# UMich-CURLY/SE3ET

Measured on AMD Instinct MI355X. Metric: point-cloud pairs/sec (fwd), SE3ET-E 5k-pt pairs, higher is better.
Workload: dtype f32

## Files before the change

### include/se3et_hip.h

```cpp
#ifndef SE3ET_HIP_H_
#define SE3ET_HIP_H_

#include <stddef.h>
#include <stdint.h>

#ifdef __cplusplus
extern "C" {
#endif

#define SE3_OK 0
#define SE3_ERR_INVALID_ARG 1
#define SE3_ERR_UNSUPPORTED 2
#define SE3_ERR_LAUNCH 3
#define SE3_ERR_WORKSPACE 4

#define SE3_MAX_BATCH 32
#define SE3_MAX_NEIGHBOR_LIMIT 64

const char* se3_version(void);
const char* se3_last_error(void);
void se3_debug_set_sinkhorn_variant(int variant);
unsigned long long se3_debug_dense_saturated_rows(int reset);
unsigned long long se3_debug_attention_saturated(int reset);
void se3_debug_kernel_timing(int enable);
// ... 34 lines not shown
                                    const int64_t* s_lengths, int batch, const void* tree_host, float radius, int limit,
                                    const int32_t* tie_rows, int64_t num_tie_rows, int max_hits, int64_t* neighbors, int* overflowed);
int64_t se3_debug_std_sort_host(const unsigned long long* keys, int64_t n, int mode);

size_t se3_grid_subsample_workspace_bytes(int64_t n, int batch);
int se3_grid_subsample(const float* points, const float* normals, int64_t n, const int64_t* lengths_host, int batch,
                       float voxel_size, float* s_points, float* s_normals, int64_t* s_lengths, void* workspace,
                       size_t workspace_bytes, void* stream);
int se3_grid_subsample_dev(const float* points, const float* normals, int64_t n_rows, const int64_t* lengths_dev, int batch,
                           float voxel_size, float* s_points, float* s_normals, int64_t* s_lengths, void* workspace,
                           size_t workspace_bytes, void* stream);

int se3_log_sinkhorn_fwd(const float* scores, const uint8_t* row_masks, const uint8_t* col_masks, const float* alpha,
                         int batch, int rows, int cols, int iterations, float inf, float* out, void* stream);
int se3_log_sinkhorn_bwd(const float* scores, const uint8_t* row_masks, const uint8_t* col_masks, const float* alpha,
                         const float* grad_out, int batch, int rows, int cols, int iterations, float inf, float* grad_scores,
                         float* grad_alpha_partial, void* stream);

size_t se3_group_norm_workspace_bytes(int64_t rows, int channels, int groups);
int se3_group_norm_fwd(const float* x, const float* x_bias, const float* residual, const float* weight, const float* bias,
                       int64_t rows, int channels, int groups, float eps, int apply_leaky_relu, float slope, float* out,
                       void* workspace, size_t workspace_bytes, void* stream);

int se3_group_norm_segments_fwd(const float* x, const float* x_bias, const float* residual, const float* weight,
                                const float* bias, int64_t rows, int channels, int groups,
                                const int64_t* segment_row_offsets_host, int num_segments, float eps, int apply_leaky_relu,
                                float slope, float* out, void* workspace, size_t workspace_bytes, void* stream);
size_t se3_group_norm_bwd_workspace_bytes(int channels);
int se3_group_norm_segments_bwd(const float* x, const float* x_bias, const float* residual, const float* weight, const float* bias,
                                const float* grad_out, int64_t rows, int channels, int groups, const int64_t* segment_row_offsets_host,
                                int num_segments, float eps, int apply_leaky_relu, float slope, float* grad_x, float* grad_residual,
                                float* grad_params, void* workspace, size_t workspace_bytes, void* stream);

size_t se3_group_norm_stats_workspace_bytes(int channels);
int se3_group_norm_stats(const float* x, const float* in_affine, float in_slope, const float* x_bias, const float* weight, const float* bias,
                         int64_t rows, int channels, int groups, const int64_t* segment_row_offsets_host, int num_segments, float eps,
                         float* affine_out, void* workspace, size_t workspace_bytes, void* stream);
int se3_group_norm_apply(const float* x, const float* affine_a, float slope_a, const float* affine_b, float slope_b, const float* residual,
                         const float* residual_affine, float final_slope, int64_t rows, int channels,
                         const int64_t* segment_row_offsets_host, int num_segments, int blocked_layout, float* out, void* stream);
int se3_group_norm_apply_amax(const float* x, const float* affine_a, float slope_a, const float* affine_b, float slope_b, const float* residual,
                              const float* residual_affine, float final_slope, int64_t rows, int channels,
                              const int64_t* segment_row_offsets_host, int num_segments, int blocked_layout, float* out, float* amax_out,
                              void* stream);
size_t se3_dense_norm_workspace_bytes(int groups);
int se3_dense_norm_fwd(const float* x, int64_t rows, int in_features, const float* in_affine_a, float in_slope_a, const float* in_affine_b,
                       float in_slope_b, const void* weight_pieces, int out_features, const float* linear_bias, const float* norm_weight,
                       const float* norm_bias, int groups, float eps, const int64_t* segment_row_offsets_host, int num_segments, float* out,
                       float* affine_out, void* workspace, size_t workspace_bytes, void* stream);
int se3_dense_residual_fwd(const float* x, int64_t rows, int in_features, const float* in_affine_a, float in_slope_a, const float* in_affine_b,
                           float in_slope_b, const void* weight_pieces, const float* affine, const float* x2, int in_features2,
                           const void* weight_pieces2, const float* affine2, const float* residual, int out_features, float final_slope,
                           const int64_t* segment_row_offsets_host, int num_segments, float* out, void* stream);
int se3_linear_stream(const float* x, int64_t rows, int in_features, int64_t x_row_stride, const void* weight_pieces, const float* bias,
                      int out_features, int apply_relu, float* out, int64_t out_row_stride, void* stream);
int se3_linear_stream_transposed(const float* x, int64_t rows, int in_features, int64_t x_row_stride, const void* weight_pieces,
                                 const float* bias, int out_features, int block_rows, float* out_t, int64_t ld, void* stream);

int se3_add_layer_norm_fwd(const float* hidden, const float* hidden_bias, const float* residual, const float* weight,
                           const float* bias, int64_t rows, int64_t residual_rows, int channels, float eps, float* out,
                           void* stream);
int se3_add_layer_norm_bwd(const float* hidden, const float* hidden_bias, const float* residual, const float* weight,
                           const float* grad_out, int64_t rows, int64_t residual_rows, int channels, float eps, float* grad_hidden,
                           float* grad_params, void* stream);

size_t se3_linear_weight_pieces_bytes(int out_features, int in_features);
int se3_linear_split_weights_f16(const float* weight, int out_features, int in_features, void* pieces, void* stream);
int se3_linear_f16(const float* x, int64_t rows, int in_features, int64_t x_row_stride, const void* weight_pieces, const float* bias,
                   int out_features, int apply_relu, float* out, int64_t out_row_stride, void* stream);

int se3_gather_rows_padded(const float* x, const int64_t* idx, int64_t n, int64_t m, int64_t width, float* out,
                           void* stream);
int se3_neighbor_max_pool(const float* x, const int64_t* idx, int64_t n, int64_t m, int nn, int64_t width, float* out,
                          void* stream);
int se3_neighbor_max_pool_bwd(const float* x, const int64_t* idx, const float* dout, int64_t n, int64_t m, int nn, int64_t width,
                              float* dx, void* stream);
int se3_anchor_max(const float* x, int num_anchors, int64_t rows, int channels, int64_t anchor_stride, int64_t row_stride,
                   float* out, void* stream);

int se3_kpconv_so3_gather(const float* q_pts, const float* s_pts, const int64_t* idx, const float* x,
                          const float* kernel_points_host, const int64_t* kidx_host, const int64_t* ridx_host, float sigma,
                          int64_t num_queries, int64_t num_support, int num_neighbors, int in_channels, float* G,
                          void* stream);
int se3_kpconv_so3_gather_bwd(const float* q_pts, const float* s_pts, const int64_t* idx, const float* dG,
                              const float* kernel_points_host, const int64_t* kidx_host, const int64_t* ridx_host, float sigma,
                              int64_t num_queries, int64_t num_support, int num_neighbors, int in_channels, float* dx, void* stream);
int se3_kpconv_so3_gather_bwd_fixed(const float* q_pts, const float* s_pts, const int64_t* idx, const float* dG,
                                    const float* kernel_points_host, const int64_t* kidx_host, const int64_t* ridx_host, float sigma,
                                    int64_t num_queries, int64_t num_support, int num_neighbors, int in_channels, const float* max_abs_dG,
                                    long long* dx_fixed, void* stream);
int se3_kpconv_fixed_to_float(const long long* dx_fixed, int64_t count, const float* max_abs_dG, int64_t num_queries, float* dx, void* stream);
int se3_fixed_to_float(const long long* fixed, int64_t count, const float* bound, int64_t terms, int growth, float* out, void* stream);
int se3_neighbor_max_pool_bwd_fixed(const float* x, const int64_t* idx, const float* dout, int64_t n, int64_t m, int nn, int64_t width,
                                    const float* max_abs_dout, long long* dx_fixed, void* stream);
int se3_scatter_add_rows_fixed(const float* g, const int64_t* idx, int64_t n, int64_t m, int64_t width, const float* max_abs_g,
                               long long* dx_fixed, void* stream);
int64_t se3_add_layer_norm_bwd_blocks(int64_t rows);
int se3_add_layer_norm_bwd_partials(const float* hidden, const float* hidden_bias, const float* residual, const float* weight,
                                    const float* grad_out, int64_t rows, int64_t residual_rows, int channels, float eps, float* grad_hidden,
                                    float* grad_params_partials, void* stream);

size_t se3_kpconv_neighbor_table_bytes(int64_t num_queries, int num_neighbors);
int se3_kpconv_neighbor_table(const float* q_pts, const float* s_pts, const int64_t* idx, const float* kernel_points_dev, float sigma,
                              int64_t num_queries, int64_t num_support, int num_neighbors, void* table, size_t table_bytes, void* stream);
size_t se3_kpconv_weight_pieces_bytes(int in_channels, int out_channels);
int se3_kpconv_split_weights_f16(const float* weights, int in_channels, int out_channels, void* pieces, void* stream);
// ... 334 lines not shown
```

### se3et_amd/csrc/dense_norm.hip

```cpp
#include "common.h"
#include "group_norm.h"

namespace {

using f16x8 = __attribute__((ext_vector_type(8))) _Float16;
using f16x4 = __attribute__((ext_vector_type(4))) _Float16;
using f32x16 = __attribute__((ext_vector_type(16))) float;
using f32x4 = __attribute__((ext_vector_type(4))) float;
using u32x4 = __attribute__((ext_vector_type(4))) unsigned;
using i32x4 = __attribute__((ext_vector_type(4))) int;

__device__ unsigned long long g_dense_saturated_rows = 0;

template <int CTRL>
__device__ __forceinline__ float dpp_f32(float v) {
  return __builtin_bit_cast(float, __builtin_amdgcn_update_dpp(0, __builtin_bit_cast(int, v), CTRL, 0xf, 0xf, true));
}

constexpr int kHeaderB = 256;
constexpr int kRowB = 80;

struct DenseArgs {
  const float* x;
  const float* in_affine[2];
// ... 768 lines not shown
    default: plain_launch<4, 1, 1, 1>(a, transposed, grid, st); break;
  }
  SE3_CHECK_LAUNCH("linear_stream");
  return SE3_OK;
}

int linear_stream(const float* x, int64_t rows, int K, int64_t x_rs, const void* weight_pieces, const float* bias, int N, int relu, float* out,
                  int64_t out_rs, int t_rows, int64_t t_ld, void* stream, int seg_channels = 0, int64_t seg_stride = 0) {
  const int64_t lim = (1ll << 29) - 1;
  const bool transposed = t_rows > 0;
  const bool fits = rows >= 0 && x_rs > 0 && rows * x_rs <= lim &&
                    (transposed ? (rows / t_rows) * (int64_t)N * t_ld <= lim : rows * (out_rs > N ? out_rs : (int64_t)N) <= lim);
  if (fits || seg_channels > 0 || !x || !out || N <= 0) return linear_stream_one(x, rows, K, x_rs, weight_pieces, bias, N, relu, out, out_rs, t_rows, t_ld, stream, seg_channels, seg_stride);
  int64_t step;
  if (transposed) {
    SE3_REQUIRE(rows % t_rows == 0 && t_ld >= t_rows, SE3_ERR_INVALID_ARG, "linear_stream: transposed output blocks of %d rows", t_rows);
    const int64_t per_block = std::max((int64_t)t_rows * x_rs, (int64_t)N * t_ld);
    SE3_REQUIRE(per_block <= lim, SE3_ERR_UNSUPPORTED, "linear_stream: one transposed block of %d rows exceeds 2 GB", t_rows);
    step = lim / per_block * t_rows;
  } else {
    SE3_REQUIRE(out_rs >= N, SE3_ERR_INVALID_ARG, "linear_stream: out row stride %lld", (long long)out_rs);
    step = lim / std::max(x_rs, out_rs) / 256 * 256;
    SE3_REQUIRE(step > 0, SE3_ERR_UNSUPPORTED, "linear_stream: row strides %lld / %lld too large", (long long)x_rs, (long long)out_rs);
  }
  for (int64_t r0 = 0; r0 < rows; r0 += step) {
    const int64_t n = std::min(step, rows - r0);
    float* o = transposed ? out + (r0 / t_rows) * (int64_t)N * t_ld : out + r0 * out_rs;
    const int rc = linear_stream_one(x + r0 * x_rs, n, K, x_rs, weight_pieces, bias, N, relu, o, out_rs, t_rows, t_ld, stream);
    if (rc != SE3_OK) return rc;
  }
  return SE3_OK;
}
}

extern "C" int se3_linear_stream(const float* x, int64_t rows, int in_features, int64_t x_row_stride, const void* weight_pieces, const float* bias,
                                 int out_features, int apply_relu, float* out, int64_t out_row_stride, void* stream) {
  return linear_stream(x, rows, in_features, x_row_stride, weight_pieces, bias, out_features, apply_relu, out, out_row_stride, 0, 0, stream);
}

extern "C" int se3_linear_stream_transposed(const float* x, int64_t rows, int in_features, int64_t x_row_stride, const void* weight_pieces,
                                            const float* bias, int out_features, int block_rows, float* out_t, int64_t ld, void* stream) {
  SE3_REQUIRE(block_rows > 0, SE3_ERR_INVALID_ARG, "linear_stream_transposed: block_rows %d", block_rows);
  return linear_stream(x, rows, in_features, x_row_stride, weight_pieces, bias, out_features, 0, out_t, 0, block_rows, ld, stream);
}


extern "C" int se3_linear_stream_segments(const float* x, int64_t rows, int in_features, int seg_channels, int64_t seg_stride,
                                          const void* weight_pieces, const float* bias, int out_features, int apply_relu, float* out,
                                          int64_t out_row_stride, void* stream) {
  SE3_REQUIRE(seg_channels > 0, SE3_ERR_INVALID_ARG, "linear_stream_segments: seg_channels %d", seg_channels);
  return linear_stream(x, rows, in_features, seg_channels, weight_pieces, bias, out_features, apply_relu, out, out_row_stride, 0, 0, stream,
                       seg_channels, seg_stride);
}
```

### se3et_amd/modules/e2pn/blocks_epn.py

```python
import math

import torch
import torch.nn as nn

from ... import functional as SF
from ... import tables


def _check_epn_config(config):
    ok = (config.kanchor == 6 and config.quotient_factor == 4 and config.num_kernel_points == 15
          and config.non_sep_conv and config.rot_by_permute and config.equiv_mode_kp
          and config.fixed_kernel_points == 'center' and config.KP_influence == 'linear'
          and config.aggregation_mode == 'sum' and not getattr(config, 'epn_kernel', False)
          and not getattr(config, 'ignore_steer_constraint', False))
    if not ok:
        raise NotImplementedError('the HIP E2PN path implements the SE3ET configuration only '
                                  '(kanchor=6, quotient_factor=4, 15 kernel points, non_sep_conv, rot_by_permute)')


class KPConvInterSO3(nn.Module):
    def __init__(self, kernel_size, kanchor, in_channels, out_channels, KP_extent, radius, KP_influence='linear',
                 aggregation_mode='sum', deformable=False, modulated=False, epn_kernel=False, equiv_mode_kp=False,
                 non_sep_conv=False, rot_by_permute=False, fixed_kernel_points='center', quotient_factor=1,
                 ignore_steer_constraint=False, gather_by_idxing=False):
# ... 73 lines not shown
        self.mlp = nn.Linear(in_dim, out_dim, bias=bias)

    def forward(self, x):
        return SF.linear(x, self.mlp.weight, self.mlp.bias)


class KPConvInterSO3Block(nn.Module):
    def __init__(self, block_name, in_dim, out_dim, radius, sigma, group_norm, config):
        super().__init__()
        _check_epn_config(config)
        self.block_name, self.in_dim, self.out_dim = block_name, in_dim, out_dim
        self.conv = KPConvInterSO3(config.num_kernel_points, config.kanchor, in_dim, out_dim, sigma, radius,
                                   config.KP_influence, config.aggregation_mode, epn_kernel=config.epn_kernel,
                                   equiv_mode_kp=config.equiv_mode_kp, non_sep_conv=config.non_sep_conv,
                                   rot_by_permute=config.rot_by_permute, fixed_kernel_points=config.fixed_kernel_points,
                                   quotient_factor=config.quotient_factor,
                                   ignore_steer_constraint=config.ignore_steer_constraint,
                                   gather_by_idxing=config.gather_by_idxing)
        self.norm = GroupNormEPN(group_norm, out_dim)

    def forward(self, x, q_pts, s_pts, neighb_inds):
        return self.norm(self.conv(q_pts, s_pts, neighb_inds, x), leaky_slope=0.1)


class SimpleBlockEPN(nn.Module):
    def __init__(self, block_name, in_dim, out_dim, radius, sigma, group_norm, config):
        super().__init__()
        self.block_name, self.in_dim, self.out_dim = block_name, in_dim, out_dim
        self.interso3 = KPConvInterSO3Block(block_name, in_dim, out_dim, radius, sigma, group_norm, config)
        self.norm = GroupNormEPN(group_norm, out_dim)

    def forward(self, x, q_pts, s_pts, neighb_inds):
        if (SF.PENDING_NORM and not SF.AG.needs_grad(x, self.interso3.conv.weights, self.norm.norm.weight) and x.is_cuda
                and self.out_dim in (16, 32, 64, 128, 256, 512, 1024)):
            y = self.interso3.norm.pending(self.interso3.conv(q_pts, s_pts, neighb_inds, x), 0.1)
            return SF.norm_apply(self.norm.pending(y, 0.1))
        return self.norm(self.interso3(x, q_pts, s_pts, neighb_inds), leaky_slope=0.1)


class ResnetBottleneckBlockEPN(nn.Module):
    def __init__(self, block_name, in_dim, out_dim, radius, sigma, group_norm, config):
        super().__init__()
        self.block_name, self.in_dim, self.out_dim = block_name, in_dim, out_dim
        bn = getattr(config, 'batch_norm_momentum', 0.99)
        mid = out_dim // 4
        self.unary1 = UnaryBlockEPN(in_dim, mid, group_norm, bn) if in_dim != mid else nn.Identity()
        self.interso3 = KPConvInterSO3Block(block_name, mid, mid, radius, sigma, group_norm, config)
        self.norm = GroupNormEPN(group_norm, mid)
        self.unary2 = UnaryBlockEPN(mid, out_dim, group_norm, bn, no_relu=True)
        self.skip_conv = UnaryBlockEPN(in_dim, out_dim, group_norm, bn, no_relu=True) if in_dim != out_dim else nn.Identity()

    def _recompute_pays(self, rows):
        k = self.unary2.in_dim + (0 if isinstance(self.skip_conv, nn.Identity) else self.skip_conv.in_dim)
        return k <= 192 and (k != 128 or rows >= 100000)

    def _forward_pending(self, x, q_pts, s_pts, neighb_inds):
        skip = x
        if not isinstance(self.unary1, nn.Identity):
            conv = self.interso3.conv
            x = SF.norm_apply(self.unary1.pending(x), blocked=True,
                              union=SF.kpconv_takes_union(q_pts, s_pts, conv.in_channels, conv.out_channels))
        y = self.interso3.norm.pending(self.interso3.conv(q_pts, s_pts, neighb_inds, x), 0.1)
        y = self.norm.pending(y, 0.1)
        if 'strided' in self.block_name:
            skip = SF.neighbor_max_pool(skip, neighb_inds)
        if self.unary2.no_relu and self._recompute_pays(y.raw.numel() // y.raw.shape[-1]) and (
                isinstance(self.skip_conv, nn.Identity) or (self.skip_conv.no_relu and SF._ops.norm_weight_nonzero(self.skip_conv.norm.norm.weight))):
            aff2 = self.unary2.stats(y)
            if isinstance(self.skip_conv, nn.Identity):
                return SF.dense_residual(y, self.unary2.mlp.weight, aff2, residual=skip, final_slope=0.1)
            skip = skip.contiguous()
            return SF.dense_residual(y, self.unary2.mlp.weight, aff2, shortcut=(skip, self.skip_conv.mlp.weight, self.skip_conv.stats(skip)),
                                     final_slope=0.1)
        if not isinstance(self.skip_conv, nn.Identity):
            skip = self.skip_conv.pending(skip)
        return SF.norm_apply(self.unary2.pending(y), residual=skip, final_slope=0.1)

    def forward(self, x, q_pts, s_pts, neighb_inds):
        if (SF.PENDING_NORM and not SF.AG.needs_grad(x, self.interso3.conv.weights, self.norm.norm.weight) and self.unary2.pending_ok(x.new_empty((0, self.unary2.in_dim)))
                and all(isinstance(u, nn.Identity) or u.pending_ok(x) for u in (self.unary1, self.skip_conv))
                and self.unary2.in_dim in (16, 32, 64, 128, 256, 512, 1024)):
            return self._forward_pending(x, q_pts, s_pts, neighb_inds)
        skip = x
        x = self.unary1(x)
        x = self.interso3(x, q_pts, s_pts, neighb_inds)
        x = self.norm(x, leaky_slope=0.1)
        if 'strided' in self.block_name:
            skip = SF.neighbor_max_pool(skip, neighb_inds)
        skip = self.skip_conv(skip)
        return self.unary2(x, residual=skip, final_slope=0.1)


class InvOutBlockEPN(nn.Module):

    def __init__(self, block_name, in_dim, config):
        super().__init__()
        if config.att_pooling or config.att_permute:
            raise NotImplementedError('InvOutBlockEPN (HIP): attention pooling is not part of the SE3ET hot path')
        self.block_name, self.in_dim = block_name, in_dim

    def forward(self, x, q_pts=None, s_pts=None, neighb_inds=None):
        return SF.anchor_max(x)


class LiftBlockEPN(nn.Module):
    def __init__(self, block_name, in_dim, config):
        super().__init__()
# ... 5 lines not shown
```

### se3et_amd/ops.py

```python
import ctypes
import os
import threading

import torch

from .caches import CACHE_EPOCH, Derived, Workspace, _Shared, also_clear, clear_caches, clear_weight_caches, validate_weight_caches
from ._lib import CONSTANTS, check, lib
from .stacking import PAIR_MAX_PAIRS, device_offsets, exclusive_offsets, to_device


_HAS_BLAS_SWITCH = hasattr(torch.backends.cuda, 'preferred_blas_library')
if _HAS_BLAS_SWITCH:
    torch.backends.cuda.preferred_blas_library('cublas')
_BLAS_SWITCH_LOCK = threading.Lock()
_BIG_GEMM_FLOP = 2.0e9


def mm(a, b):
    big = 2.0 * a.shape[0] * a.shape[1] * b.shape[1] > _BIG_GEMM_FLOP
    if _HAS_BLAS_SWITCH and big and (b.stride(-1) == 1 or a.shape[1] <= 32):
        with _BLAS_SWITCH_LOCK:
            torch.backends.cuda.preferred_blas_library('cublaslt')
            try:
                return torch.mm(a, b)
# ... 643 lines not shown
        ring[2] += 1
    slot = ring[0][ring[1]:ring[1] + 1]
    ring[1] += 1
    return slot, (ring, ring[2], ring[1] - 1)


def _amax_live(blocked):
    if blocked.amax is None or blocked.amax_tag is None:
        return blocked.amax
    ring, gen, pos = blocked.amax_tag
    return blocked.amax if ring[2] == gen else None


def _kpconv_union_pays(Cin, Cout, same_cloud):
    return KPCONV_UNION_ALL or (Cout <= 64 and (same_cloud or Cout <= 32))


def dense_norm_ok(x, weight, groups):
    raw = x.raw if isinstance(x, Pending) else x
    if torch.is_grad_enabled() and (raw.requires_grad or weight.requires_grad):
        return False
    N, K = weight.shape
    return (raw.is_cuda and raw.dtype == torch.float32 and weight.dtype == torch.float32 and weight.is_contiguous() and raw.is_contiguous()
            and raw.shape[-1] == K and 32 <= K <= 1024 and K & (K - 1) == 0 and (N in (32, 64, 128) or N % 256 == 0) and N % groups == 0
            and N // groups in (1, 2, 4, 8, 16, 32) and N <= 4096
            and raw.data_ptr() % 16 == 0)


def dense_norm(x, weight, linear_bias, norm_weight, norm_bias, groups, eps, segments=None):
    pend = x if isinstance(x, Pending) else Pending(x, [], [], segments)
    raw = _req(pend.raw, torch.float32, 'x')
    if len(pend.affines) > 2:
        raise RuntimeError('dense_norm: at most two pending stages')
    segments = pend.segments if segments is None else segments
    N, K = weight.shape
    rows = raw.numel() // K
    stream = _stream()
    Wp = _linear_weight_pieces(weight, stream)
    nseg = 1 if segments is None else len(segments) - 1
    out = torch.empty(raw.shape[:-1] + (N,), dtype=torch.float32, device=raw.device)
    affine = torch.empty((nseg, 2, N), dtype=torch.float32, device=raw.device)
    ws = _ws_dense.get(raw.device, stream.value, lib().se3_dense_norm_workspace_bytes(int(groups)))
    aa = pend.affines + [None, None]
    sl = pend.slopes + [1.0, 1.0]
    with _timed('dense', 4.0 * rows * (K + N)):
        _check_counters(lib().se3_dense_norm_fwd(raw.data_ptr(), rows, K, aa[0].data_ptr() if aa[0] is not None else None, float(sl[0]),
                                       aa[1].data_ptr() if aa[1] is not None else None, float(sl[1]), Wp.data_ptr(), N,
                                       linear_bias.data_ptr() if linear_bias is not None else None, norm_weight.data_ptr(), norm_bias.data_ptr(),
                                       int(groups), float(eps), _i64_array(segments) if nseg > 1 else None, nseg, out.data_ptr(),
                                       affine.data_ptr(), ws.data_ptr(), ws.numel(), stream), 'se3_dense_norm_fwd', ws)
    return Pending(out, [affine], [1.0], segments)


def dense_stats(x, weight, linear_bias, norm_weight, norm_bias, groups, eps, segments=None):
    pend = x if isinstance(x, Pending) else Pending(x, [], [], segments)
    raw = _req(pend.raw, torch.float32, 'x')
    if len(pend.affines) > 2:
        raise RuntimeError('dense_stats: at most two pending stages')
    segments = pend.segments if segments is None else segments
    N, K = weight.shape
    rows = raw.numel() // K
    stream = _stream()
    Wp = _linear_weight_pieces(weight, stream)
    nseg = 1 if segments is None else len(segments) - 1
    affine = torch.empty((nseg, 2, N), dtype=torch.float32, device=raw.device)
    ws = _ws_dense.get(raw.device, stream.value, lib().se3_dense_norm_workspace_bytes(int(groups)))
    aa = pend.affines + [None, None]
    sl = pend.slopes + [1.0, 1.0]
    with _timed('dense', 4.0 * rows * K):
        _check_counters(lib().se3_dense_norm_fwd(raw.data_ptr(), rows, K, aa[0].data_ptr() if aa[0] is not None else None, float(sl[0]),
                                       aa[1].data_ptr() if aa[1] is not None else None, float(sl[1]), Wp.data_ptr(), N,
                                       linear_bias.data_ptr() if linear_bias is not None else None, norm_weight.data_ptr(), norm_bias.data_ptr(),
                                       int(groups), float(eps), _i64_array(segments) if nseg > 1 else None, nseg, None,
                                       affine.data_ptr(), ws.data_ptr(), ws.numel(), stream), 'se3_dense_norm_fwd (statistics only)', ws)
    return affine


_nonzero_norms = Derived(256, weights=True)


def norm_weight_nonzero(weight):
    key = (weight.data_ptr(), weight.device.index, tuple(weight.shape))
    hit = _nonzero_norms.lookup(weight, key)
    return hit if hit is not None else _nonzero_norms.store(weight, key, bool((weight.detach().abs() > 1e-30).all()))


def dense_residual(x, weight, affine, residual=None, shortcut=None, final_slope=1.0, segments=None):
    pend = x if isinstance(x, Pending) else Pending(x, [], [], segments)
    raw = _req(pend.raw, torch.float32, 'x')
    if len(pend.affines) > 2:
        raise RuntimeError('dense_residual: at most two pending stages')
    segments = pend.segments if segments is None else segments
    N, K = weight.shape
    rows = raw.numel() // K
    stream = _stream()
    Wp = _linear_weight_pieces(weight, stream)
    nseg = 1 if segments is None else len(segments) - 1
    if tuple(affine.shape) != (nseg, 2, N):
        raise RuntimeError('dense_residual: affine table %s for %d segment(s) x %d features' % (tuple(affine.shape), nseg, N))
    out = torch.empty(raw.shape[:-1] + (N,), dtype=torch.float32, device=raw.device)
    x2p = wp2 = aff2 = resp = None
    K2 = 0
    if shortcut is not None:
        x2, w2, aff2t = shortcut
        x2 = _req(x2, torch.float32, 'shortcut input')
        K2 = w2.shape[1]
        if w2.shape[0] != N or x2.numel() != rows * K2 or tuple(aff2t.shape) != (nseg, 2, N) or residual is not None:
            raise RuntimeError('dense_residual: shortcut layer shapes')
        x2p, wp2, aff2 = x2.data_ptr(), _linear_weight_pieces(w2, stream).data_ptr(), aff2t.data_ptr()
    elif residual is not None:
        residual = _req(residual, torch.float32, 'residual')
        if residual.numel() != rows * N:
            raise RuntimeError('dense_residual: residual shape %s' % (tuple(residual.shape),))
        resp = residual.data_ptr()
    aa = pend.affines + [None, None]
    sl = pend.slopes + [1.0, 1.0]
    with _timed('dense', 4.0 * rows * (K + K2 + N + (N if resp is not None else 0))):
# ... 1424 lines not shown
```

Measured before the change: 449.0.

## Compute dense group-norm statistics from the input Gram matrix instead of the output

Adds a statistics-only path that accumulates a centred, split-f16 MFMA Gram matrix (x^T x) and column sums of the transformed input per chunk. It merges these per segment and derives the per-channel mean and variance of W x analytically in a finalize kernel. This avoids running the full K->N GEMM when only the normalisation affine is needed, which is cheaper when N is several times K. A heuristic picks this path for large row counts with K <= 128, and the recompute threshold in the EPN block is also lowered. The cost is extra numerical risk from the Gram-form variance (handled with centring and exponent scaling) and three kernel launches instead of one.

```diff
diff --git a/include/se3et_hip.h b/include/se3et_hip.h
--- a/include/se3et_hip.h
+++ b/include/se3et_hip.h
@@ -110,6 +110,11 @@
                            float in_slope_b, const void* weight_pieces, const float* affine, const float* x2, int in_features2,
                            const void* weight_pieces2, const float* affine2, const float* residual, int out_features, float final_slope,
                            const int64_t* segment_row_offsets_host, int num_segments, float* out, void* stream);
+size_t se3_dense_gram_stats_workspace_bytes(int in_features);
+int se3_dense_gram_stats_fwd(const float* x, int64_t rows, int in_features, const float* in_affine_a, float in_slope_a, const float* in_affine_b,
+                             float in_slope_b, const float* weight, int out_features, const float* linear_bias, const float* norm_weight,
+                             const float* norm_bias, int groups, float eps, const int64_t* segment_row_offsets_host, int num_segments,
+                             float* affine_out, void* workspace, size_t workspace_bytes, void* stream);
 int se3_linear_stream(const float* x, int64_t rows, int in_features, int64_t x_row_stride, const void* weight_pieces, const float* bias,
                       int out_features, int apply_relu, float* out, int64_t out_row_stride, void* stream);
 int se3_linear_stream_transposed(const float* x, int64_t rows, int in_features, int64_t x_row_stride, const void* weight_pieces,
diff --git a/se3et_amd/csrc/dense_norm.hip b/se3et_amd/csrc/dense_norm.hip
--- a/se3et_amd/csrc/dense_norm.hip
+++ b/se3et_amd/csrc/dense_norm.hip
@@ -844,3 +844,511 @@
   return linear_stream(x, rows, in_features, seg_channels, weight_pieces, bias, out_features, apply_relu, out, out_row_stride, 0, 0, stream,
                        seg_channels, seg_stride);
 }
+
+
+namespace {
+
+constexpr int kGramHdr = 8;
+constexpr size_t kGramPartialBudgetB = 32u << 20;
+
+size_t gram_partial_floats(int K) { return (size_t)kGramHdr + 2 * (size_t)K + (size_t)K * K; }
+size_t gram_segment_floats(int K) { return (size_t)kGramHdr + (size_t)K + (size_t)K * K; }
+
+struct GramArgs {
+  const float* x;
+  const float* in_affine[2];
+  float in_slope[2];
+  int K;
+  float* part;
+  SegTable T;
+};
+
+__device__ __forceinline__ f16x4 lds_read_tr16(const unsigned char* p) {
+  typedef __fp16 fp16x4 __attribute__((__vector_size__(4 * sizeof(__fp16))));
+  return __builtin_bit_cast(f16x4, __builtin_amdgcn_ds_read_tr16_b64_v4f16((__attribute__((address_space(3))) fp16x4*)(p)));
+}
+
+template <int NF>
+__global__ __launch_bounds__(256, NF >= 128 ? 2 : 3) void dense_norm_gram_kernel(const GramArgs a) {
+  constexpr int FB = NF > 128 ? 128 : NF;
+  constexpr int SR = 4096 / NF, NSUB = SR / 16, NFB = NF / 32;
+  constexpr int RS = NF == 32 ? 4 : 1;
+  constexpr int WG = NF == 32 ? 1 : 2, TT = FB / 32 / WG;
+  constexpr int kBlockB = SR * 64, kPieceB = NFB * kBlockB, kBufB = 2 * kPieceB;
+  constexpr int BT0 = NF > FB ? FB / 32 : 0;
+  static_assert(kBufB == 16384, "one step is 4096 values in two f16 pieces");
+  __shared__ __align__(16) unsigned char lds[2 * kBufB];
+  __shared__ __align__(16) float affl[2][2][NF];
+  __shared__ __align__(16) float cvec[NF];
+  __shared__ float psum[256];
+  __shared__ int amax_bits;
+  const int tid = threadIdx.x, lane = tid & 63, wave = __builtin_amdgcn_readfirstlane(tid >> 6);
+  const int K = a.K;
+  const int nb = K / FB, bi = blockIdx.y / nb, bj = blockIdx.y - bi * nb;
+  long long r0, r1;
+  chunk_rows(a.T, blockIdx.x, r0, r1);
+  if (r1 < r0) r1 = r0;
+  const int seg = seg_of_chunk(a.T, blockIdx.x);
+  const int nrows = (int)(r1 - r0);
+  const int nsteps = (nrows + SR - 1) / SR;
+  const int stages = (a.in_affine[0] != nullptr) + (a.in_affine[1] != nullptr);
+  auto gfeat = [&](int s) { return s < FB ? bi * FB + s : bj * FB + (s - FB); };
+  for (int st = 0; st < stages; st++)
+    for (int i = tid; i < 2 * NF; i += 256) {
+      const int half = i / NF, s = i - half * NF;
+      affl[st][half][s] = a.in_affine[st][(size_t)seg * 2 * K + half * K + gfeat(s)];
+    }
+  if (tid == 0) amax_bits = 0;
+  const int c8 = tid & 7;
+  int urow[4], sfeat[4], xoff[4], loff[4];
+#pragma unroll
+  for (int u = 0; u < 4; u++) {
+    const int rest = u * 32 + (tid >> 3);
+    urow[u] = rest % SR;
+    const int fblk = rest / SR;
+    sfeat[u] = fblk * 32 + 4 * c8;
+    xoff[u] = (urow[u] * K + gfeat(sfeat[u])) * 4;
+    loff[u] = fblk * kBlockB + urow[u] * 64 + c8 * 8;
+  }
+  const __amdgpu_buffer_rsrc_t xrs =
+      __builtin_amdgcn_make_buffer_rsrc(const_cast<float*>(a.x + (nrows > 0 ? r0 : 0) * K), 0, nrows * K * 4, 0x00020000);
+  auto request = [&](int step, f32x4 (&v)[4]) {
+    const int soff = step * (SR * K * 4);
+#pragma unroll
+    for (int u = 0; u < 4; u++) v[u] = __builtin_bit_cast(f32x4, __builtin_amdgcn_raw_buffer_load_b128(xrs, xoff[u], soff, 0));
+  };
+  auto transformed = [&](int u, const f32x4& raw) {
+    f32x4 t = raw;
+    if (stages > 0) {
+      t = t * *reinterpret_cast<const f32x4*>(&affl[0][0][sfeat[u]]) + *reinterpret_cast<const f32x4*>(&affl[0][1][sfeat[u]]);
+#pragma unroll
+      for (int e = 0; e < 4; e++) t[e] = t[e] > 0.f ? t[e] : t[e] * a.in_slope[0];
+    }
+    if (stages > 1) {
+      t = t * *reinterpret_cast<const f32x4*>(&affl[1][0][sfeat[u]]) + *reinterpret_cast<const f32x4*>(&affl[1][1][sfeat[u]]);
+#pragma unroll
+      for (int e = 0; e < 4; e++) t[e] = t[e] > 0.f ? t[e] : t[e] * a.in_slope[1];
+    }
+    return t;
+  };
+  f32x4 ra[4], rb[4];
+  request(0, ra);
+  __syncthreads();
+  float* scr = reinterpret_cast<float*>(lds);
+#pragma unroll
+  for (int u = 0; u < 4; u++) {
+    f32x4 t = transformed(u, ra[u]);
+    if (urow[u] >= nrows) t = f32x4{0.f, 0.f, 0.f, 0.f};
+    *reinterpret_cast<f32x4*>(&scr[(u * 32 + (tid >> 3)) * 32 + 4 * c8]) = t;
+  }
+  __syncthreads();
+  constexpr int PARTS = 256 / NF;
+  const int pcol = tid % NF, ppart = tid / NF, pfb = pcol >> 5, pcc = pcol & 31, cnt = nrows < SR ? nrows : SR;
+  {
+    float sum = 0.f;
+#pragma unroll
+    for (int r = 0; r < 16; r++) sum += scr[(pfb * SR + ppart * 16 + r) * 32 + pcc];
+    psum[ppart * NF + pcol] = sum;
+  }
+  __syncthreads();
+  if (tid < NF) {
+    float sum = 0.f;
+#pragma unroll
+    for (int q = 0; q < PARTS; q++) sum += psum[q * NF + tid];
+    cvec[tid] = cnt > 0 ? sum / (float)cnt : 0.f;
+  }
+  __syncthreads();
+  {
+    const float cm = cvec[pcol];
+    int mb = 0;
+#pragma unroll
+    for (int r = 0; r < 16; r++) {
+      const int bits = __builtin_bit_cast(int, __builtin_fabsf(scr[(pfb * SR + ppart * 16 + r) * 32 + pcc] - cm)) & 0x7fffffff;
+      mb = ppart * 16 + r < cnt ? max(mb, bits) : mb;
+    }
+    atomicMax(&amax_bits, mb);
+  }
+  __syncthreads();
+  const int eh = (amax_bits >> 23) & 0xff;
+  const int E = (eh == 0 || eh >= 255 || (eh >= 123 && eh <= 133)) ? 0 : max(-100, min(100, 133 - eh));
+  const float sE = __builtin_ldexpf(1.f, E);
+  const bool count_here = bi == bj;
+  f32x4 S[4];
+#pragma unroll
+  for (int u = 0; u < 4; u++) S[u] = f32x4{0.f, 0.f, 0.f, 0.f};
+
+  auto stage = [&](int buf, int step, const f32x4 (&v)[4]) {
+    unsigned char* img = lds + buf * kBufB;
+    unsigned long long odd = 0;
+    f32x4 tv[4];
+#pragma unroll
+    for (int u = 0; u < 4; u++) {
+      f32x4 d = transformed(u, v[u]) - *reinterpret_cast<const f32x4*>(&cvec[sfeat[u]]);
+      if (step * SR + urow[u] >= nrows) d = f32x4{0.f, 0.f, 0.f, 0.f};
+      S[u] += d;
+      d *= sE;
+      tv[u] = d;
+      const float m = fmaxf(fmaxf(__builtin_fabsf(d[0]), __builtin_fabsf(d[1])), fmaxf(__builtin_fabsf(d[2]), __builtin_fabsf(d[3])));
+      odd |= __builtin_amdgcn_ballot_w64(!(m < 32768.f));
+    }
+    if (__builtin_expect(odd == 0, 1)) {
+#pragma unroll
+      for (int u = 0; u < 4; u++) {
+        f16x4 hi, lo;
+#pragma unroll
+        for (int e = 0; e < 4; e++) {
+          hi[e] = (_Float16)tv[u][e];
+          lo[e] = (_Float16)(2.f * (tv[u][e] - (float)hi[e]));
+        }
+        *reinterpret_cast<f16x4*>(img + loff[u]) = hi;
+        *reinterpret_cast<f16x4*>(img + kPieceB + loff[u]) = lo;
+      }
+      return;
+    }
+    int saturated = 0;
+#pragma unroll 1
+    for (int u = 0; u < 4; u++) {
+      f32x4 t = tv[0];
+      int lo_off = loff[0], sf = sfeat[0];
+#pragma unroll
+      for (int uu = 1; uu < 4; uu++) {
+        t = u == uu ? tv[uu] : t;
+        lo_off = u == uu ? loff[uu] : lo_off;
+        sf = u == uu ? sfeat[uu] : sf;
+      }
+      bool flag = false;
+      f16x4 hi, lo;
+#pragma unroll
+      for (int e = 0; e < 4; e++) {
+        const bool nonfinite = (__float_as_uint(t[e]) & 0x7f800000u) == 0x7f800000u;
+        flag |= nonfinite || __builtin_fabsf(t[e]) > 65000.f;
+        float te = fminf(fmaxf(t[e], -65000.f), 65000.f);
+        te = nonfinite ? __builtin_bit_cast(float, 0x7fc00000) : te;
+        hi[e] = (_Float16)te;
+        lo[e] = (_Float16)(2.f * (te - (float)hi[e]));
+      }
+      *reinterpret_cast<f16x4*>(img + lo_off) = hi;
+      *reinterpret_cast<f16x4*>(img + kPieceB + lo_off) = lo;
+      unsigned long long rowsf = __builtin_amdgcn_ballot_w64(flag && count_here && sf < FB);
+      rowsf |= rowsf >> 4;
+      rowsf |= rowsf >> 2;
+      rowsf |= rowsf >> 1;
+      saturated += __builtin_popcountll(rowsf & 0x0101010101010101ull);
+    }
+    if (saturated && lane == 0) atomicAdd(&g_dense_saturated_rows, (unsigned long long)saturated);
+  };
+
+  const int wi = WG == 2 ? wave >> 1 : 0, wj = WG == 2 ? wave & 1 : 0;
+  const int i32 = lane & 31, h = lane >> 5;
+  const int tr_off = (8 * h + ((lane & 15) >> 2)) * 64 + 32 * ((lane >> 4) & 1) + 8 * (lane & 3);
+  f32x16 acc[TT][TT];
+#pragma unroll
+  for (int ti = 0; ti < TT; ti++)
+#pragma unroll
+    for (int tj = 0; tj < TT; tj++)
+#pragma unroll
+      for (int v = 0; v < 16; v++) acc[ti][tj][v] = 0.f;
+  auto multiply = [&](int buf) {
+    const unsigned char* img = lds + buf * kBufB + tr_off;
+#pragma unroll
+    for (int s0 = 0; s0 < NSUB; s0 += RS) {
+      const int sub = RS > 1 ? s0 + wave : s0;
+      const unsigned char* rows16 = img + sub * (16 * 64);
+      f16x8 ah[TT], bh[TT], bl[TT];
+#pragma unroll
+      for (int t = 0; t < TT; t++) {
+        const unsigned char* pa = rows16 + (wi * TT + t) * kBlockB;
+        const unsigned char* pb = rows16 + (BT0 + wj * TT + t) * kBlockB;
+        const f16x4 a0 = lds_read_tr16(pa), a1 = lds_read_tr16(pa + 4 * 64);
+        const f16x4 b0 = lds_read_tr16(pb), b1 = lds_read_tr16(pb + 4 * 64);
+        const f16x4 l0 = lds_read_tr16(pb + kPieceB), l1 = lds_read_tr16(pb + kPieceB + 4 * 64);
+        ah[t] = __builtin_shufflevector(a0, a1, 0, 1, 2, 3, 4, 5, 6, 7);
+        bh[t] = __builtin_shufflevector(b0, b1, 0, 1, 2, 3, 4, 5, 6, 7);
+        bl[t] = __builtin_shufflevector(l0, l1, 0, 1, 2, 3, 4, 5, 6, 7);
+      }
+#pragma unroll
+      for (int ti = 0; ti < TT; ti++)
+#pragma unroll
+        for (int tj = 0; tj < TT; tj++) {
+          acc[ti][tj] = __builtin_amdgcn_mfma_f32_32x32x16_f16(ah[ti], bh[tj], acc[ti][tj], 0, 0, 0);
+          acc[ti][tj] = __builtin_amdgcn_mfma_f32_32x32x16_f16(ah[ti], bl[tj], acc[ti][tj], 0, 0, 0);
+        }
+    }
+  };
+
+  request(0, ra);
+  request(1, rb);
+  stage(0, 0, ra);
+#pragma unroll
+  for (int u = 0; u < 4; u++) ra[u] = rb[u];
+  request(2, rb);
+  __syncthreads();
+#pragma unroll 1
+  for (int s = 0; s < nsteps; s++) {
+    multiply(s & 1);
+    stage((s + 1) & 1, s + 1, ra);
+#pragma unroll
+    for (int u = 0; u < 4; u++) ra[u] = rb[u];
+    request(s + 3, rb);
+    __syncthreads();
+  }
+
+  float* P = a.part + (size_t)blockIdx.x * (kGramHdr + 2 * (size_t)K + (size_t)K * K);
+  if constexpr (RS > 1) {
+    float* red = reinterpret_cast<float*>(lds);
+#pragma unroll
+    for (int v = 0; v < 16; v++) red[(wave * 16 + v) * 64 + lane] = acc[0][0][v];
+    __syncthreads();
+    if (wave == 0) {
+#pragma unroll
+      for (int v = 0; v < 16; v++)
+        acc[0][0][v] = ((red[v * 64 + lane] + red[(16 + v) * 64 + lane]) + red[(32 + v) * 64 + lane]) + red[(48 + v) * 64 + lane];
+    }
+  }
+  if (RS == 1 || wave == 0) {
+    float* Q = P + kGramHdr + 2 * K;
+#pragma unroll
+    for (int ti = 0; ti < TT; ti++)
+#pragma unroll
+      for (int tj = 0; tj < TT; tj++)
+#pragma unroll
+        for (int v = 0; v < 16; v++) {
+          const int i = bi * FB + (wi * TT + ti) * 32 + (v & 3) + 8 * (v >> 2) + 4 * h;
+          const int j = bj * FB + (wj * TT + tj) * 32 + i32;
+          Q[(size_t)i * K + j] = __builtin_ldexpf(acc[ti][tj][v], -2 * E);
+        }
+  }
+  float* sred = reinterpret_cast<float*>(lds + kBufB);
+#pragma unroll
+  for (int u = 0; u < 4; u++) *reinterpret_cast<f32x4*>(&sred[(u * 32 + (tid >> 3)) * 32 + 4 * c8]) = S[u];
+  __syncthreads();
+  {
+    float s = 0.f;
+#pragma unroll
+    for (int r = 0; r < 16; r++) s += sred[(pfb * SR + ppart * 16 + r) * 32 + pcc];
+    psum[ppart * NF + pcol] = s;
+  }
+  __syncthreads();
+  if (tid < FB && bi == bj) {
+    float s = 0.f;
+#pragma unroll
+    for (int q = 0; q < PARTS; q++) s += psum[q * NF + tid];
+    P[kGramHdr + bi * FB + tid] = cvec[tid];
+    P[kGramHdr + K + bi * FB + tid] = s;
+  }
+  if (tid == 0 && blockIdx.y == 0) P[0] = (float)nrows;
+}
+
+__global__ __launch_bounds__(256) void dense_norm_gram_merge_kernel(const float* __restrict__ part, int K, SegTable T, float* __restrict__ seg_stats) {
+  const int seg = blockIdx.y;
+  int cb0 = T.chunk_begin[0], cb1 = T.chunk_begin[1];
+#pragma unroll
+  for (int s = 1; s < kGNMaxSegments; s++)
+    if (seg == s) {
+      cb0 = T.chunk_begin[s];
+      cb1 = T.chunk_begin[s + 1];
+    }
+  const int idx = blockIdx.x * 256 + threadIdx.x, i = idx / K, j = idx - i * K;
+  const size_t PS = kGramHdr + 2 * (size_t)K + (size_t)K * K;
+  float n = 0.f, mi = 0.f, mj = 0.f, M = 0.f;
+  for (int p0 = cb0; p0 < cb1; p0 += 16) {
+    float np[16], ci[16], cj[16], si[16], sj[16], qv[16];
+#pragma unroll
+    for (int b = 0; b < 16; b++) {
+      const bool live = p0 + b < cb1;
+      const float* P = part + (size_t)(live ? p0 + b : cb1 - 1) * PS;
+      np[b] = live ? P[0] : 0.f;
+      ci[b] = P[kGramHdr + i];
+      cj[b] = P[kGramHdr + j];
+      si[b] = P[kGramHdr + K + i];
+      sj[b] = P[kGramHdr + K + j];
+      qv[b] = P[kGramHdr + 2 * K + idx];
+    }
+#pragma unroll
+    for (int b = 0; b < 16; b++) {
+      if (np[b] == 0.f) continue;
+      const float inv = 1.f / np[b];
+      const float mpi = ci[b] + si[b] * inv, mpj = cj[b] + sj[b] * inv;
+      const float m2 = qv[b] - si[b] * sj[b] * inv;
+      if (n == 0.f) {
+        n = np[b];
+        mi = mpi;
+        mj = mpj;
+        M = m2;
+      } else {
+        const float nn = n + np[b], f = np[b] / nn, di = mpi - mi, dj = mpj - mj;
+        M += m2 + di * dj * n * f;
+        mi += di * f;
+        mj += dj * f;
+        n = nn;
+      }
+    }
+  }
+  float* O = seg_stats + seg * ((size_t)kGramHdr + K + (size_t)K * K);
+  O[kGramHdr + K + idx] = M;
+  if (j == 0) O[kGramHdr + i] = mi;
+  if (idx == 0) O[0] = n;
+}
+
+constexpr int kGramFinRows = 16;
+__global__ __launch_bounds__(256) void dense_norm_gram_finalize_kernel(const float* __restrict__ seg_stats, int K, const float* __restrict__ W, int N,
+                                                                       const float* __restrict__ xb, const float* __restrict__ gw,
+                                                                       const float* __restrict__ gb, int groups, float eps, float* __restrict__ affine) {
+  extern __shared__ __align__(16) float wl[];
+  __shared__ float redq[8][32], redm[8][32];
+  const int seg = blockIdx.y, c0 = blockIdx.x * 32, tid = threadIdx.x;
+  const float* O = seg_stats + seg * ((size_t)kGramHdr + K + (size_t)K * K);
+  const float* mu = O + kGramHdr;
+  const float* M = O + kGramHdr + K;
+  const int PK = K < 256 ? K : 256, P4 = PK >> 2, WS = PK + 4;
+  float* mt = wl + 32 * WS;
+  const int cl = tid & 31, s = tid >> 5;
+  const float* w = wl + cl * WS;
+  const float* wrow = W + (size_t)(c0 + cl) * K;
+  float q = 0.f, m = 0.f;
+  for (int j0 = 0; j0 < K; j0 += PK) {
+    __syncthreads();
+    for (int idx = tid; idx < 32 * P4; idx += 256) {
+      const int r = idx / P4, k4 = idx - r * P4;
+      *reinterpret_cast<f32x4*>(&wl[r * WS + 4 * k4]) = *reinterpret_cast<const f32x4*>(&W[(size_t)(c0 + r) * K + j0 + 4 * k4]);
+    }
+    for (int i0 = 0; i0 < K; i0 += kGramFinRows) {
+      __syncthreads();
+      for (int idx = tid; idx < kGramFinRows * P4; idx += 256) {
+        const int r = idx / P4, k4 = idx - r * P4;
+        *reinterpret_cast<f32x4*>(&mt[r * PK + 4 * k4]) = *reinterpret_cast<const f32x4*>(&M[(size_t)(i0 + r) * K + j0 + 4 * k4]);
+      }
+      const float w0 = wrow[i0 + s], w1 = wrow[i0 + s + 8];
+      __syncthreads();
+      const float* m0 = mt + s * PK;
+      const float* m1 = mt + (s + 8) * PK;
+      f32x4 t0 = {0.f, 0.f, 0.f, 0.f}, t1 = t0;
+#pragma unroll 8
+      for (int j4 = 0; j4 < P4; j4++) {
+        const f32x4 wv = *reinterpret_cast<const f32x4*>(&w[4 * j4]);
+        t0 += *reinterpret_cast<const f32x4*>(&m0[4 * j4]) * wv;
+        t1 += *reinterpret_cast<const f32x4*>(&m1[4 * j4]) * wv;
+      }
+      q += w0 * ((t0[0] + t0[1]) + (t0[2] + t0[3]));
+      q += w1 * ((t1[0] + t1[1]) + (t1[2] + t1[3]));
+      if (j0 == 0) m += w0 * mu[i0 + s] + w1 * mu[i0 + s + 8];
+    }
+  }
+  redq[s][cl] = q;
+  redm[s][cl] = m;
+  __syncthreads();
+  if (tid >= 64) return;
+  q = m = 0.f;
+#pragma unroll
+  for (int ss = 0; ss < 8; ss++) {
+    q += redq[ss][cl];
+    m += redm[ss][cl];
+  }
+  const int col = c0 + cl, cpg = N / groups;
+  const float bias = xb ? xb[col] : 0.f;
+  WF wv = {O[0], m + bias, q < 0.f ? 0.f : q};
+  for (int d = 1; d < cpg; d <<= 1) {
+    const WF o = {__shfl_xor(wv.n, d), __shfl_xor(wv.mean, d), __shfl_xor(wv.m2, d)};
+    wv = wf_merge(wv, o);
+  }
+  const float mean = wv.mean, rstd = 1.0f / sqrtf(wv.m2 / fmaxf(wv.n, 1.f) + eps);
+  const int first = (tid & 63) & ~(cpg - 1);
+  const float mean0 = __shfl(mean, first), rstd0 = __shfl(rstd, first);
+  if (tid < 32) {
+    const float scale = rstd0 * gw[col];
+    affine[(size_t)seg * 2 * N + col] = scale;
+    affine[(size_t)seg * 2 * N + N + col] = gb[col] + (bias - mean0) * scale;
+  }
+}
+
+size_t gram_finalize_lds_bytes(int K) {
+  const int PK = K < 256 ? K : 256;
+  return (size_t)(32 * (PK + 4) + kGramFinRows * PK) * sizeof(float);
+}
+
+int gram_chunk_target(int K) {
+  const int nblk = K > 128 ? (K / 128) * (K / 128) : 1;
+  int64_t want = (K > 64 ? 512 : 768) / nblk;
+  const int64_t fit = (int64_t)(kGramPartialBudgetB / (gram_partial_floats(K) * sizeof(float)));
+  if (want > fit) want = fit;
+  return (int)(want < 1 ? 1 : want);
+}
+int gram_chunks(int64_t rows, int K, const int64_t* segment_row_offsets_host, int num_segments, SegTable& T) {
+  const int NF = K > 128 ? 256 : K, SR = 4096 / NF;
+  T = SegTable{};
+  T.n = num_segments;
+  T.quantum = SR;
+  int64_t tiles = 0;
+  for (int s = 0; s < num_segments; s++) {
+    const int64_t b0 = num_segments == 1 ? 0 : segment_row_offsets_host[s], b1 = num_segments == 1 ? rows : segment_row_offsets_host[s + 1];
+    if (!(b1 > b0 && b0 >= 0 && b1 <= rows)) return -1;
+    tiles += se3_cdiv(b1 - b0, SR);
+  }
+  const int64_t tiles_per_chunk = se3_cdiv(tiles, gram_chunk_target(K));
+  int chunks = 0;
+  for (int s = 0; s < num_segments; s++) {
+    const int64_t b0 = num_segments == 1 ? 0 : segment_row_offsets_host[s], b1 = num_segments == 1 ? rows : segment_row_offsets_host[s + 1];
+    T.row_begin[s] = b0;
+    T.row_begin[s + 1] = b1;
+    T.chunk_begin[s] = chunks;
+    chunks += (int)se3_cdiv(se3_cdiv(b1 - b0, SR), tiles_per_chunk);
+    T.chunk_begin[s + 1] = chunks;
+  }
+  if (!(T.row_begin[0] == 0 && T.row_begin[num_segments] == rows && chunks <= gram_chunk_target(K) + kGNMaxSegments)) return -1;
+  return chunks;
+}
+}
+
+extern "C" size_t se3_dense_gram_stats_workspace_bytes(int in_features) {
+  const int K = in_features;
+  if (K < 32 || K > 512) return 0;
+  return ((size_t)(gram_chunk_target(K) + kGNMaxSegments) * gram_partial_floats(K) + (size_t)kGNMaxSegments * gram_segment_floats(K)) * sizeof(float);
+}
+
+extern "C" int se3_dense_gram_stats_fwd(const float* x, int64_t rows, int in_features, const float* in_affine_a, float in_slope_a,
+                                        const float* in_affine_b, float in_slope_b, const float* weight, int out_features,
+                                        const float* linear_bias, const float* norm_weight, const float* norm_bias, int groups, float eps,
+                                        const int64_t* segment_row_offsets_host, int num_segments, float* affine_out, void* workspace,
+                                        size_t workspace_bytes, void* stream) {
+  SE3_REQUIRE(x && weight && norm_weight && norm_bias && affine_out && workspace, SE3_ERR_INVALID_ARG, "dense_gram_stats: null pointer");
+  const int K = in_features, N = out_features;
+  SE3_REQUIRE(K >= 32 && K <= 512 && (K & (K - 1)) == 0 && N >= 32 && N % 32 == 0, SE3_ERR_UNSUPPORTED,
+              "dense_gram_stats: %d -> %d features (in: a power of two 32..512; out: a multiple of 32)", K, N);
+  SE3_REQUIRE(rows >= 1 && rows * K < (1ll << 29) && groups >= 1 && N % groups == 0, SE3_ERR_INVALID_ARG, "dense_gram_stats: rows %lld groups %d",
+              (long long)rows, groups);
+  {
+    const int cpg = N / groups;
+    SE3_REQUIRE(cpg <= 32 && (cpg & (cpg - 1)) == 0, SE3_ERR_UNSUPPORTED, "dense_gram_stats: %d channels per group (a power of two <= 32)", cpg);
+  }
+  SE3_REQUIRE(num_segments >= 1 && num_segments <= kGNMaxSegments && (num_segments == 1 || segment_row_offsets_host), SE3_ERR_UNSUPPORTED,
+              "dense_gram_stats: %d segments (1..%d)", num_segments, kGNMaxSegments);
+  SE3_REQUIRE(((uintptr_t)x & 15) == 0 && ((uintptr_t)weight & 15) == 0 && (in_affine_a || !in_affine_b), SE3_ERR_INVALID_ARG,
+              "dense_gram_stats: x and weight must be 16-byte aligned; stage b needs stage a");
+  SE3_REQUIRE(in_slope_a >= 0.f && in_slope_a <= 1.f && in_slope_b >= 0.f && in_slope_b <= 1.f, SE3_ERR_INVALID_ARG,
+              "dense_gram_stats: LeakyReLU slopes must lie in [0, 1]");
+  SE3_REQUIRE(workspace_bytes >= se3_dense_gram_stats_workspace_bytes(K) && ((uintptr_t)workspace & 15) == 0, SE3_ERR_WORKSPACE,
+              "dense_gram_stats: workspace too small or misaligned");
+  GramArgs a{};
+  const int chunks = gram_chunks(rows, K, segment_row_offsets_host, num_segments, a.T);
+  SE3_REQUIRE(chunks > 0, SE3_ERR_INVALID_ARG, "dense_gram_stats: the segments must be non-empty, ascending and cover all %lld rows", (long long)rows);
+  a.x = x;
+  a.in_affine[0] = in_affine_a;
+  a.in_affine[1] = in_affine_b;
+  a.in_slope[0] = in_slope_a;
+  a.in_slope[1] = in_slope_b;
+  a.K = K;
+  a.part = static_cast<float*>(workspace);
+  float* seg_stats = a.part + (size_t)(gram_chunk_target(K) + kGNMaxSegments) * gram_partial_floats(K);
+  hipStream_t st = (hipStream_t)stream;
+  const int nblk = K > 128 ? (K / 128) * (K / 128) : 1;
+  const dim3 grid((unsigned)chunks, (unsigned)nblk);
+  if (K == 32) dense_norm_gram_kernel<32><<<grid, 256, 0, st>>>(a);
+  else if (K == 64) dense_norm_gram_kernel<64><<<grid, 256, 0, st>>>(a);
+  else if (K == 128) dense_norm_gram_kernel<128><<<grid, 256, 0, st>>>(a);
+  else dense_norm_gram_kernel<256><<<grid, 256, 0, st>>>(a);
+  dense_norm_gram_merge_kernel<<<dim3((unsigned)(K * K / 256), (unsigned)num_segments), 256, 0, st>>>(a.part, K, a.T, seg_stats);
+  dense_norm_gram_finalize_kernel<<<dim3((unsigned)(N / 32), (unsigned)num_segments), 256, gram_finalize_lds_bytes(K), st>>>(
+      seg_stats, K, weight, N, linear_bias, norm_weight, norm_bias, groups, eps, affine_out);
+  SE3_CHECK_LAUNCH("dense_gram_stats");
+  return SE3_OK;
+}
diff --git a/se3et_amd/modules/e2pn/blocks_epn.py b/se3et_amd/modules/e2pn/blocks_epn.py
--- a/se3et_amd/modules/e2pn/blocks_epn.py
+++ b/se3et_amd/modules/e2pn/blocks_epn.py
@@ -149,7 +149,7 @@
 
     def _recompute_pays(self, rows):
         k = self.unary2.in_dim + (0 if isinstance(self.skip_conv, nn.Identity) else self.skip_conv.in_dim)
-        return k <= 192 and (k != 128 or rows >= 100000)
+        return k <= 192 and (k != 128 or rows >= 60000)
 
     def _forward_pending(self, x, q_pts, s_pts, neighb_inds):
         skip = x
diff --git a/se3et_amd/ops.py b/se3et_amd/ops.py
--- a/se3et_amd/ops.py
+++ b/se3et_amd/ops.py
@@ -719,6 +719,44 @@
     return Pending(out, [affine], [1.0], segments)
 
 
+_DENSE_GRAM_ENV = os.environ.get('SE3_DENSE_GRAM', '1')
+DENSE_GRAM = _DENSE_GRAM_ENV != '0'
+DENSE_GRAM_ALL = _DENSE_GRAM_ENV == 'all'
+_ws_gram = Workspace(1 << 20)
+
+
+def dense_gram_ok(K, N, rows, groups):
+    return K in (32, 64, 128, 256, 512) and N % 32 == 0 and N % groups == 0 and N // groups in (1, 2, 4, 8, 16, 32) and rows * K < 1 << 29
+
+
+def _gram_stats_pays(K, N, rows, nseg):
+    return K <= 128 and ((N >= 4 * K and rows * K >= 14000000) or (N >= 2 * K and rows * K >= 28000000))
+
+
+def dense_gram_stats(x, weight, linear_bias, norm_weight, norm_bias, groups, eps, segments=None):
+    pend = x if isinstance(x, Pending) else Pending(x, [], [], segments)
+    raw = _req(pend.raw, torch.float32, 'x')
+    if len(pend.affines) > 2:
+        raise RuntimeError('dense_stats: at most two pending stages')
+    segments = pend.segments if segments is None else segments
+    weight = _req(weight, torch.float32, 'weight')
+    N, K = weight.shape
+    rows = raw.numel() // K
+    stream = _stream()
+    nseg = 1 if segments is None else len(segments) - 1
+    affine = torch.empty((nseg, 2, N), dtype=torch.float32, device=raw.device)
+    ws = _ws_gram.get(raw.device, stream.value, lib().se3_dense_gram_stats_workspace_bytes(int(K)))
+    aa = pend.affines + [None, None]
+    sl = pend.slopes + [1.0, 1.0]
+    with _timed('dense', 4.0 * rows * K):
+        check(lib().se3_dense_gram_stats_fwd(raw.data_ptr(), rows, K, aa[0].data_ptr() if aa[0] is not None else None, float(sl[0]),
+                                             aa[1].data_ptr() if aa[1] is not None else None, float(sl[1]), weight.data_ptr(), N,
+                                             linear_bias.data_ptr() if linear_bias is not None else None, norm_weight.data_ptr(),
+                                             norm_bias.data_ptr(), int(groups), float(eps), _i64_array(segments) if nseg > 1 else None, nseg,
+                                             affine.data_ptr(), ws.data_ptr(), ws.numel(), stream), 'se3_dense_gram_stats_fwd')
+    return affine
+
+
 def dense_stats(x, weight, linear_bias, norm_weight, norm_bias, groups, eps, segments=None):
     pend = x if isinstance(x, Pending) else Pending(x, [], [], segments)
     raw = _req(pend.raw, torch.float32, 'x')
@@ -727,9 +765,11 @@
     segments = pend.segments if segments is None else segments
     N, K = weight.shape
     rows = raw.numel() // K
+    nseg = 1 if segments is None else len(segments) - 1
+    if DENSE_GRAM and weight.is_contiguous() and dense_gram_ok(K, N, rows, groups) and (DENSE_GRAM_ALL or _gram_stats_pays(K, N, rows, nseg)):
+        return dense_gram_stats(pend, weight, linear_bias, norm_weight, norm_bias, groups, eps, segments)
     stream = _stream()
     Wp = _linear_weight_pieces(weight, stream)
-    nseg = 1 if segments is None else len(segments) - 1
     affine = torch.empty((nseg, 2, N), dtype=torch.float32, device=raw.device)
     ws = _ws_dense.get(raw.device, stream.value, lib().se3_dense_norm_workspace_bytes(int(groups)))
     aa = pend.affines + [None, None]
```

Result: no change. 451.9, median of 6 (+0.6%).
